# slothfulxtx/Texture-GS

Measured on AMD Instinct MI355X. Metric: fwd+bwd views/sec @800x800, 300k Gaussians + 1024^2 texture; HBM GB/s vs roofline, higher is better.
Workload: dtype f32; 1 GPU; c3: N=300000 Gaussians, cubemap 6x1024x1024x3 f32, 800x800, fwd+bwd, sh_degree 3; parallelism=views sharded dp1, view_pipeline=3 HIP streams, order=accumulate, forwards begun one view per stream ahead, grad_allreduce=none (1 GPU)

## Files before the change

### include/texgs_multiview.h

```cpp
#ifndef TEXGS_MULTIVIEW_H
#define TEXGS_MULTIVIEW_H

#include <stddef.h>
#include <stdint.h>

#include "texgs.h"

#ifdef __cplusplus
extern "C" {
#endif

#define TEXGS_SH_FLUSH_MAX_VIEWS 16

typedef struct TexGSShFlushView {
    const float* campos;
    const float* residue;
    int32_t sh_degree;
    int32_t sh_coeffs;
} TexGSShFlushView;

int texgs_sh_flush(int32_t N, int32_t K, const float* means3D, const float* shs, float* dL_dshs, float* dL_dmeans3D,
                   const TexGSShFlushView* views, int32_t count, void* stream);

#define TEXGS_BATCH_MAX_VIEWS 16

int texgs_preprocess_forward_views(const TexGSFrame* frames, const TexGSInputs* in, TexGSGeom* geoms, int32_t count, uint32_t* sums,
                                   void* stream);
int texgs_depth_sort_scan_views(const TexGSGeom* geoms, int32_t num_gaussians, int32_t count, void* stream);
int texgs_bin_sort_views(const TexGSFrame* frames, const TexGSGeom* geoms, TexGSBinning* bins, const TexGSImage* imgs, int32_t count,
                         void* stream);
int texgs_render_forward_binned(const TexGSFrame* frame, const TexGSInputs* in, const TexGSGeom* geom, const TexGSBinning* bin,
                                TexGSImage* img, void* stream);

#ifdef __cplusplus
}
#endif

#endif
```

### texture-gs_amd/csrc/abi.hip

```cpp
#include "common.h"
#include <stdio.h>
#include <stdlib.h>

#include <mutex>
#include <vector>

namespace {

thread_local char g_err[512] = "";

struct EvRec { int kid; hipEvent_t a, b; };
std::mutex g_prof_mu;
bool g_prof_on = false;
uint32_t g_prof_mask = 0xFFFFFFFFu;
std::vector<EvRec> g_prof_log;
std::vector<hipEvent_t> g_prof_free;

hipEvent_t prof_event() {
    if (!g_prof_free.empty()) { hipEvent_t e = g_prof_free.back(); g_prof_free.pop_back(); return e; }
    hipEvent_t e = nullptr;
    return hipEventCreate(&e) == hipSuccess ? e : nullptr;
}

struct ProfScope {
// ... 605 lines not shown
            if (!b.keys_unsorted || !b.keys_sorted || !b.point_list || !b.sort_temp) return fail_msg("NULL buffer in a view's TexGSBinning");
            if (b.sort_temp_bytes < sort_temp_bytes(b.num_rendered, T)) return fail_msg("sort_temp too small");
        }
        if ((imgs[v].tex_bin_count != nullptr) && frames[v].tex_res != frames[0].tex_res) return fail_msg("the views of a batch must have one tex_res");
    }
    hipStream_t s = (hipStream_t)stream;
    hipError_t st;
    const int nzw = 2 * (int)tex_bin_count(c.R);
    { ProfScope p(TEXGS_K_DUPLICATE, s); st = launch_bin_views(TEXGS_K_DUPLICATE, c, geoms, bins, imgs, count, nzw, s); }
    if (int r = launched("duplicate_with_keys (views)", st, s, frames[0].debug)) return r;
    { ProfScope p(TEXGS_K_SORT, s); st = launch_bin_views(TEXGS_K_SORT, c, geoms, bins, imgs, count, nzw, s); }
    if (int r = launched("tile sort (views)", st, s, frames[0].debug)) return r;
    { ProfScope p(TEXGS_K_RANGES, s); st = launch_bin_views(TEXGS_K_RANGES, c, geoms, bins, imgs, count, nzw, s); }
    return launched("tile_ranges (views)", st, s, frames[0].debug);
}

int texgs_render_forward_binned(const TexGSFrame* frame, const TexGSInputs* in, const TexGSGeom* geom, const TexGSBinning* bin,
                                TexGSImage* img, void* stream) {
    return render_forward_impl(frame, in, geom, bin, img, stream, true);
}

static int check_mlp(const TexGSMlp* m) {
    if (!m) return fail_msg("mlp is NULL");
    const char* what = nullptr;
    int v = 0;
    if (m->n_neurons != TEXGS_MLP_WIDTH) { what = "n_neurons must be 128"; v = m->n_neurons; }
    else if (m->n_hidden_layers < 1 || m->n_hidden_layers > TEXGS_MLP_MAX_HIDDEN_LAYERS) { what = "n_hidden_layers must be 1 or 2"; v = m->n_hidden_layers; }
    else if (m->n_in < 1 || m->n_in > TEXGS_MLP_WIDTH) { what = "n_in must be in [1,128]"; v = m->n_in; }
    else if (m->n_out < 1 || m->n_out > TEXGS_MLP_WIDTH) { what = "n_out must be in [1,128]"; v = m->n_out; }
    if (!what) return 0;
// ... 453 lines not shown
```

### texture-gs_amd/csrc/binning.hip

```cpp
#include "common.h"
#include <cstring>

namespace {

constexpr int RS_THREADS = 256;
constexpr int RS_MAX_BLOCKS = 1024;
constexpr int RS_GROUP = 32;
#ifndef RS_PER_MIN
#define RS_PER_MIN 512u
#endif

struct RadixTables {
    uint32_t* table;
    uint32_t* gtable;
};
constexpr size_t RS_ZERO_WORDS = (size_t)(RS_MAX_BLOCKS / RS_GROUP) * 256;

__device__ __forceinline__ uint32_t digit_of(uint64_t k, int shift, uint32_t mask) { return (uint32_t)(k >> shift) & mask; }

__device__ __forceinline__ void block_range(uint32_t n, uint32_t per, uint32_t& lo, uint32_t& hi) {
    lo = min(n, blockIdx.x * per);
    hi = min(n, lo + per);
}

// ... 17 lines not shown
    t.table[blockIdx.x * 256 + threadIdx.x] = c;
    if (c != 0u) atomicAdd(&t.gtable[(blockIdx.x / RS_GROUP) * 256 + threadIdx.x], c);
}

template <typename KEY>
__global__ void __launch_bounds__(RS_THREADS)
k_radix_count(const KEY* __restrict__ keys, const uint32_t* __restrict__ n_ptr, uint32_t n_max, uint32_t per, int shift,
              uint32_t mask, RadixTables t) {
    radix_count_body<KEY>(keys, n_ptr ? min(*n_ptr, n_max) : n_max, per, shift, mask, t);
}

template <typename KEY, int MODE>
__device__ __forceinline__ void radix_scatter_body(const KEY* __restrict__ keys_in, const uint32_t* __restrict__ vals_in, KEY* __restrict__ keys_out,
                uint32_t* __restrict__ vals_out, uint32_t n, uint32_t nblocks, uint32_t per, int shift,
                uint32_t mask, int bits, RadixTables t, const uint32_t* __restrict__ depth_rank,
                const uint32_t* __restrict__ id_rank) {
    __shared__ uint32_t s_wcnt[4][256];
    __shared__ uint32_t s_scan[256];
    uint32_t lo, hi;
    block_range(n, per, lo, hi);
    if (lo >= hi) return;
    const int tid = threadIdx.x, lane = tid & 63, wv = tid >> 6;
    constexpr int RB = 8;
    const uint32_t rows = (hi - lo + 63u) >> 6, rows_per_wave = (rows + 3u) >> 2;
    const uint32_t wlo = min(hi, lo + (uint32_t)wv * rows_per_wave * 64u), whi = min(hi, wlo + rows_per_wave * 64u);
    const bool single = (whi - wlo) <= 64u * RB;
    KEY kk[RB];
    uint32_t vv[RB];
    auto load_batch = [&](uint32_t b0) {
#pragma unroll
        for (int rr = 0; rr < RB; ++rr) {
// ... 36 lines not shown
#pragma unroll
        for (int rr = 0; rr < RB; ++rr)
            if (b0 + 64u * rr + lane < whi) atomicAdd(&s_wcnt[wv][digit_of(kk[rr], shift, mask)], 1u);
    }
    __syncthreads();
    {
        uint32_t run = before;
#pragma unroll
        for (int w = 0; w < 4; ++w) { const uint32_t c = s_wcnt[w][tid]; s_wcnt[w][tid] = run; run += c; }
    }
    __syncthreads();
    uint32_t* cur = s_wcnt[wv];
    for (uint32_t b0 = wlo; b0 < whi; b0 += 64u * RB) {
        if (!single) load_batch(b0);
        uint32_t dr[RB];
        if (MODE == 2) {
#pragma unroll
            for (int rr = 0; rr < RB; ++rr) {
                const bool have = b0 + 64u * rr + lane < whi;
                dr[rr] = have ? depth_rank[(uint32_t)kk[rr]] : 0u;
                vv[rr] = have ? id_rank[(uint32_t)kk[rr]] : 0u;
            }
        }
#pragma unroll
        for (int rr = 0; rr < RB; ++rr) {
            const uint32_t i = b0 + 64u * rr + lane;
            if (b0 + 64u * rr >= whi) break;
            const bool have = i < whi;
            const KEY k = kk[rr];
            const uint32_t d = have ? digit_of(k, shift, mask) : 0xFFFFFFFFu;
            unsigned long long peers = __ballot(have);
            for (int bt = 0; bt < bits; ++bt) {
                const unsigned long long m = __ballot((d >> bt) & 1u);
                peers &= ((d >> bt) & 1u) ? m : ~m;
            }
            uint32_t pos = 0u;
            if (have) {
                const uint32_t below = (uint32_t)__builtin_amdgcn_mbcnt_hi((uint32_t)(peers >> 32), __builtin_amdgcn_mbcnt_lo((uint32_t)peers, 0u));
                pos = cur[d] + below;
            }
            __builtin_amdgcn_wave_barrier();
            if (have && (peers >> lane) >> 1 == 0ull) cur[d] = pos + 1u;
            __builtin_amdgcn_wave_barrier();
            if (have) {
                if (MODE == 0) {
                    keys_out[pos] = k;
                    vals_out[pos] = vv[rr];
                } else if (MODE == 1) {
                    keys_out[pos] = k;
                } else {
                    keys_out[pos] = (KEY)(((uint64_t)k & 0xFFFFFFFF00000000ull) | (uint64_t)dr[rr]);
                    vals_out[pos] = vv[rr];
                }
            }
        }
    }
}

template <typename KEY, int MODE>
__global__ void __launch_bounds__(RS_THREADS)
k_radix_scatter(const KEY* __restrict__ keys_in, const uint32_t* __restrict__ vals_in, KEY* __restrict__ keys_out,
                uint32_t* __restrict__ vals_out, const uint32_t* __restrict__ n_ptr, uint32_t n_max, uint32_t per, int shift,
                uint32_t mask, int bits, RadixTables t, const uint32_t* __restrict__ depth_rank,
                const uint32_t* __restrict__ id_rank) {
    radix_scatter_body<KEY, MODE>(keys_in, vals_in, keys_out, vals_out, n_ptr ? min(*n_ptr, n_max) : n_max, gridDim.x, per, shift, mask,
                                  bits, t, depth_rank, id_rank);
// ... 413 lines not shown
    for (int k = 0; k < 9; ++k) { const int q = tid * per + k; v[k] = (k < per && q < nb1) ? bsum[q] : 0u; sum += v[k]; }
    uint32_t incl = sum;
#pragma unroll
    for (int d = 1; d < 64; d <<= 1) { const uint32_t o = (uint32_t)__shfl_up((int)incl, d, 64); if (lane >= d) incl += o; }
    if (lane == 63) s_w[wv] = incl;
    __syncthreads();
    uint32_t run = incl - sum;
    for (int w = 0; w < wv; ++w) run += s_w[w];
#pragma unroll
    for (int k = 0; k < 9; ++k) { const int q = tid * per + k; if (k < per && q < nb1) bsum[q] = run; run += v[k]; }
}

__global__ void __launch_bounds__(1024)
k_depth_prefix(const uint32_t* __restrict__ drange, uint32_t* __restrict__ bsum) { depth_prefix_body(drange, bsum); }

template <bool PRE>
__device__ __forceinline__ void duplicate_body(int N, int tiles_x, int T, const uint32_t* __restrict__ id_rank, const uint32_t* __restrict__ key_rank,
            const uint32_t* __restrict__ loc_rank, uint32_t* __restrict__ offs_rank, const uint32_t* __restrict__ drange, const uint32_t* __restrict__ gmap, const uint32_t* __restrict__ bsum,
            const uint32_t* __restrict__ tiles_touched, const uint2* __restrict__ rect, uint64_t* __restrict__ elems,
            uint2* __restrict__ ranges, uint32_t* __restrict__ zero_words, int num_zero_words) {
    __shared__ uint32_t s_pre[PRE ? 1 : DS_FUSED_GROUPS + 1];
    __shared__ uint32_t s_w[TG_BLOCK / 64];
    const int r = blockIdx.x * TG_BLOCK + threadIdx.x;
    for (int k = r; k < T; k += (int)gridDim.x * TG_BLOCK) ranges[k] = make_uint2(0u, 0u);
    for (int k = r; k < num_zero_words; k += (int)gridDim.x * TG_BLOCK) zero_words[k] = 0u;
    const uint32_t d_lo = drange[DR_LO], d_scale = drange[DR_SCALE], d_nb = drange[DR_NB];
    uint32_t my_group = 0u, my_off = 0u;
    if (r < N) { my_group = gmap[depth_bin(key_rank[r], d_lo, d_scale, d_nb)]; my_off = loc_rank[r]; }
    uint32_t my_pre = 0u;
    if constexpr (PRE) {
        if (r < N) my_pre = bsum[my_group];
    } else {
        const int tid = threadIdx.x, lane = tid & 63, wv = tid >> 6, nb1 = (int)drange[DR_GROUPS] + 1;
        for (int q = tid; q < nb1; q += TG_BLOCK) s_pre[q] = bsum[q];
        __syncthreads();
// ... 8 lines not shown
        uint32_t run = incl - sum;
        for (int w = 0; w < wv; ++w) run += s_w[w];
        for (int k = 0; k < per; ++k) { const int q = tid * per + k; if (q < nb1) { const uint32_t c = s_pre[q]; s_pre[q] = run; run += c; } }
        __syncthreads();
        my_pre = s_pre[my_group];
    }
    if (r >= N) return;
    uint32_t off = my_off + my_pre;
    offs_rank[r] = off;
    const uint32_t id = id_rank[r];
    if (tiles_touched[id] == 0u) return;
    const uint2 rc = rect[id];
    const uint32_t x0 = rc.x & 0xffffu, y0 = rc.x >> 16, x1 = rc.y & 0xffffu, y1 = rc.y >> 16;
    for (uint32_t y = y0; y < y1; ++y)
        for (uint32_t x = x0; x < x1; ++x)
            elems[off++] = ((uint64_t)(y * (uint32_t)tiles_x + x) << 32) | (uint64_t)(uint32_t)r;
}

template <bool PRE>
__global__ void __launch_bounds__(TG_BLOCK)
k_duplicate(int N, int tiles_x, int T, const uint32_t* __restrict__ id_rank, const uint32_t* __restrict__ key_rank,
            const uint32_t* __restrict__ loc_rank, uint32_t* __restrict__ offs_rank, const uint32_t* __restrict__ drange, const uint32_t* __restrict__ gmap, const uint32_t* __restrict__ bsum,
            const uint32_t* __restrict__ tiles_touched, const uint2* __restrict__ rect, uint64_t* __restrict__ elems,
            uint2* __restrict__ ranges, uint32_t* __restrict__ zero_words, int num_zero_words) {
    duplicate_body<PRE>(N, tiles_x, T, id_rank, key_rank, loc_rank, offs_rank, drange, gmap, bsum, tiles_touched, rect, elems, ranges,
                        zero_words, num_zero_words);
}

__device__ __forceinline__ void ranges_body(uint32_t D, const uint64_t* __restrict__ keys, uint2* __restrict__ ranges) {
    const uint32_t i = blockIdx.x * TG_BLOCK + threadIdx.x;
    if (i >= D) return;
    const uint32_t cur = (uint32_t)(keys[i] >> 32);
    if (i == 0) ranges[cur].x = 0;
    else {
        const uint32_t prev = (uint32_t)(keys[i - 1] >> 32);
        if (cur != prev) { ranges[prev].y = i; ranges[cur].x = i; }
    }
    if (i == D - 1) ranges[cur].y = D;
}

__global__ void __launch_bounds__(TG_BLOCK)
// ... 147 lines not shown
}

__global__ void __launch_bounds__(DS_THREADS)
k_depth_group_sort_views(BinViews a, int N, int gmax) {
    const BinView& w = a.v[blockIdx.y];
    const GaussScratch gs = gauss_scratch(w.scan_temp, N);
    depth_group_sort_body(N, gs.gpos, gs.drange, gs.pair_a, gs.key_b, gs.val_b, w.tiles_touched, gs.loc_b, gs.bsum, gmax);
}

__global__ void __launch_bounds__(1024)
k_depth_prefix_views(BinViews a, int N) {
    const GaussScratch gs = gauss_scratch(a.v[blockIdx.y].scan_temp, N);
    depth_prefix_body(gs.drange, gs.bsum);
}

template <bool PRE>
__global__ void __launch_bounds__(TG_BLOCK)
k_duplicate_views(BinViews a, int N, int tiles_x, int T, int num_zero_words) {
    const BinView& w = a.v[blockIdx.y];
    if (w.D == 0u) {
        for (int k = blockIdx.x * TG_BLOCK + threadIdx.x; k < T; k += (int)gridDim.x * TG_BLOCK) w.ranges[k] = make_uint2(0u, 0u);
        return;
    }
    const GaussScratch gs = gauss_scratch(w.scan_temp, N);
    duplicate_body<PRE>(N, tiles_x, T, gs.val_b, gs.key_b, gs.loc_b, w.offsets, gs.drange, gs.gmap, gs.bsum, w.tiles_touched, w.rect,
                        w.keys_unsorted, w.ranges, reinterpret_cast<uint32_t*>(w.sort_temp), num_zero_words);
}

__global__ void __launch_bounds__(RS_THREADS)
k_radix_count_views(BinViews a, int pass, int from_tmp, int shift, uint32_t mask) {
    const BinView& w = a.v[blockIdx.y];
    uint32_t blocks, per;
    pass_geometry(w.D, blocks, per);
    if (w.D == 0u || blockIdx.x >= blocks) return;
    radix_count_body<uint64_t>(from_tmp ? sort_tmp_of(w) : w.keys_unsorted, w.D, per, shift, mask,
                               tables_at(reinterpret_cast<uint32_t*>(w.sort_temp), pass, TILE_PASSES_MAX, 0));
}

template <int MODE>
__global__ void __launch_bounds__(RS_THREADS)
k_radix_scatter_views(BinViews a, int N, int pass, int from_tmp, int to_tmp, int shift, uint32_t mask, int bits) {
    const BinView& w = a.v[blockIdx.y];
    uint32_t blocks, per;
    pass_geometry(w.D, blocks, per);
    if (w.D == 0u || blockIdx.x >= blocks) return;
    const uint64_t* src = from_tmp ? sort_tmp_of(w) : w.keys_unsorted;
    const RadixTables t = tables_at(reinterpret_cast<uint32_t*>(w.sort_temp), pass, TILE_PASSES_MAX, 0);
    if (MODE == 2) {
        const GaussScratch gs = gauss_scratch(w.scan_temp, N);
        radix_scatter_body<uint64_t, 2>(src, nullptr, w.keys_sorted, w.point_list, w.D, blocks, per, shift, mask, bits, t, gs.key_b, gs.val_b);
    } else {
        radix_scatter_body<uint64_t, 1>(src, nullptr, to_tmp ? sort_tmp_of(w) : w.keys_unsorted, nullptr, w.D, blocks, per, shift, mask, bits, t,
                                        nullptr, nullptr);
    }
}

__global__ void __launch_bounds__(TG_BLOCK)
k_ranges_views(BinViews a) {
    const BinView& w = a.v[blockIdx.y];
    if (w.D != 0u) ranges_body(w.D, w.keys_sorted, w.ranges);
}

__global__ void __launch_bounds__(1024)
k_tile_order_views(BinViews a, uint32_t T, int num_zero_words) {
    const BinView& w = a.v[blockIdx.y];
    tile_order_body(T, w.ranges, w.tile_order, w.zero_words, w.zero_words ? num_zero_words : 0);
}

// ... 2 lines not shown
    memset(&a, 0, sizeof(a));
    for (int v = 0; v < count; ++v) {
        BinView& w = a.v[v];
        w.depth = reinterpret_cast<const uint32_t*>(g[v].depth); w.tiles_touched = g[v].tiles_touched;
        w.rect = reinterpret_cast<const uint2*>(g[v].rect); w.offsets = g[v].offsets; w.scan_temp = g[v].scan_temp;
        if (b) {
            w.keys_unsorted = b[v].keys_unsorted; w.keys_sorted = b[v].keys_sorted; w.point_list = b[v].point_list;
            w.ranges = reinterpret_cast<uint2*>(b[v].ranges); w.tile_order = b[v].tile_order; w.sort_temp = b[v].sort_temp;
            w.D = b[v].num_rendered;
        }
        if (img) w.zero_words = img[v].tex_bin_count;
    }
    return a;
}

}

hipError_t launch_depth_sort_scan_views(const TexGSGeom* g, int N, int count, hipStream_t s) {
    if (N <= 0 || count <= 0) return hipSuccess;
    const BinViews a = bin_views(g, nullptr, nullptr, count);
    const int nblk = (N + TG_BLOCK - 1) / TG_BLOCK;
    const int blocks = (N + DS_PER - 1) / DS_PER;
    const int lb = depth_log2_bins(N);
    const int gmax = depth_max_groups(N, 1 << lb);
    hipLaunchKernelGGL(k_depth_count_views, dim3(blocks, count), dim3(DS_THREADS), 0, s, a, N, nblk, lb);
    hipLaunchKernelGGL(k_depth_scatter_views, dim3(blocks, count), dim3(DS_THREADS), 0, s, a, N, nblk, lb);
    hipLaunchKernelGGL(k_depth_group_sort_views, dim3(gmax + (N + (int)DS_COPY - 1) / (int)DS_COPY, count), dim3(DS_THREADS), 0, s, a, N, gmax);
    if (gmax > DS_FUSED_GROUPS) hipLaunchKernelGGL(k_depth_prefix_views, dim3(1, count), dim3(1024), 0, s, a, N);
    return hipGetLastError();
}

hipError_t launch_bin_views(int stage, const CamConst& c, const TexGSGeom* g, const TexGSBinning* b, const TexGSImage* img, int count,
                            int num_zero_words, hipStream_t s) {
    if (c.N <= 0 || count <= 0) return hipSuccess;
    const BinViews a = bin_views(g, b, img, count);
    const uint32_t T = (uint32_t)(c.tiles_x * c.tiles_y);
    uint32_t dmax = 0u;
    for (int v = 0; v < count; ++v) dmax = b[v].num_rendered > dmax ? b[v].num_rendered : dmax;
    const int nblocks = (c.N + TG_BLOCK - 1) / TG_BLOCK;
    const bool pre = depth_max_groups(c.N, 1 << depth_log2_bins(c.N)) > DS_FUSED_GROUPS;
    const int hdr = (int)(zero_header_bytes(TILE_PASSES_MAX, 0) / 4);
    if (stage == TEXGS_K_DUPLICATE) {
        if (pre) hipLaunchKernelGGL(k_duplicate_views<true>, dim3(nblocks, count), dim3(TG_BLOCK), 0, s, a, c.N, c.tiles_x, (int)T, hdr);
        else hipLaunchKernelGGL(k_duplicate_views<false>, dim3(nblocks, count), dim3(TG_BLOCK), 0, s, a, c.N, c.tiles_x, (int)T, hdr);
    }
    if (stage == TEXGS_K_SORT && dmax > 0u) {
        const int tb = tile_bits(T);
        const int npass = (tb + 7) / 8;
        if (npass > TILE_PASSES_MAX) return hipErrorInvalidValue;
        uint32_t blocks = 1u;
        for (int v = 0; v < count; ++v) {
            uint32_t bv, per;
            pass_geometry(b[v].num_rendered, bv, per);
            blocks = bv > blocks ? bv : blocks;
        }
        int from_tmp = 0, shift = 32, left = tb;
        for (int pass = 0; pass < npass; ++pass) {
            const int bits = (left + (npass - pass) - 1) / (npass - pass);
            const uint32_t mask = (1u << bits) - 1u;
            hipLaunchKernelGGL(k_radix_count_views, dim3(blocks, count), dim3(RS_THREADS), 0, s, a, pass, from_tmp, shift, mask);
            if (pass == npass - 1) {
                hipLaunchKernelGGL(k_radix_scatter_views<2>, dim3(blocks, count), dim3(RS_THREADS), 0, s, a, c.N, pass, from_tmp, 0, shift, mask, bits);
            } else {
                const int to_tmp = from_tmp ? 0 : 1;
                hipLaunchKernelGGL(k_radix_scatter_views<1>, dim3(blocks, count), dim3(RS_THREADS), 0, s, a, c.N, pass, from_tmp, to_tmp, shift, mask, bits);
                from_tmp = to_tmp;
            }
            shift += bits; left -= bits;
        }
    }
    if (stage == TEXGS_K_RANGES) {
        if (dmax > 0u) hipLaunchKernelGGL(k_ranges_views, dim3((dmax + TG_BLOCK - 1) / TG_BLOCK, count), dim3(TG_BLOCK), 0, s, a);
        hipLaunchKernelGGL(k_tile_order_views, dim3(1, count), dim3(1024), 0, s, a, T, num_zero_words);
    }
    return hipGetLastError();
}

hipError_t launch_depth_sort_scan(const TexGSGeom* g, int N, hipStream_t s) {
    if (N <= 0) return hipSuccess;
    const GaussScratch gs = gauss_scratch(g->scan_temp, N);
    const int nblk = (N + TG_BLOCK - 1) / TG_BLOCK;
    const int blocks = (N + DS_PER - 1) / DS_PER;
// ... 111 lines not shown
```

### texture-gs_amd/csrc/common.h

```cpp
#pragma once
#include <hip/hip_runtime.h>
#include <stdint.h>
#include "texgs.h"
#include "texgs_optim.h"
#include "texgs_multiview.h"
#include "texgs_mlp.h"
#include "texgs_present.h"
#include "texgs_ingest.h"
#include "texgs_surface.h"
#include "texgs_lpips.h"
#include "texgs_lpips_grad.h"
#include "texgs_params.h"
#include "texgs_retexture.h"

#define TG_NEAR_Z        0.2f
#define TG_LOWPASS       0.3f
#define TG_FRUSTUM_CLAMP 1.3f
#define TG_ALPHA_MAX     0.99f
#define TG_ALPHA_MIN     (1.0f / 255.0f)
#define TG_T_EPS         1e-4f
#define TG_PLANE_EPS     5e-2f
#define TG_DEN_MIN       0.2f
#define TG_MA_MIN        1e-20f
#define TG_SH_C0         0.28209479177387814f
// ... 39 lines not shown
hipError_t launch_sh_flush(int N, int K, const float* means3D, const float* shs, float* dL_dshs, float* dL_dmeans3D,
                           const TexGSShFlushView* views, int count, hipStream_t s);
hipError_t launch_mark_visible(const TexGSFrame* f, const float* means3D, uint8_t* visible, hipStream_t s);
hipError_t launch_depth_sort_scan(const TexGSGeom* g, int N, hipStream_t s);
uint32_t* bin_block_sums_ptr(const TexGSGeom* g, int N);
uint32_t* bin_header_ptr(const TexGSGeom* g, int N, int* words);
size_t scan_temp_bytes(int N);
size_t sort_temp_bytes(uint32_t D, uint32_t T);
hipError_t launch_duplicate(const CamConst& c, const TexGSGeom* g, TexGSBinning* b, hipStream_t s);
hipError_t launch_sort(const CamConst& c, const TexGSGeom* g, TexGSBinning* b, hipStream_t s);
hipError_t launch_ranges(const CamConst& c, TexGSBinning* b, uint32_t* zero_words, int num_zero_words, hipStream_t s);
hipError_t launch_preprocess_fwd_views(const TexGSFrame* f, const TexGSInputs* in, TexGSGeom* g, int count, uint32_t* sums, hipStream_t s);
hipError_t launch_depth_sort_scan_views(const TexGSGeom* g, int N, int count, hipStream_t s);
hipError_t launch_bin_views(int stage, const CamConst& c, const TexGSGeom* g, const TexGSBinning* b, const TexGSImage* img, int count,
                            int num_zero_words, hipStream_t s);
hipError_t launch_render_fwd(const CamConst& c, const TexGSFrame* f, const TexGSInputs* in, const TexGSGeom* g,
                       const TexGSBinning* b, TexGSImage* img, hipStream_t s);
size_t tex_bin_count(int R);
bool tex_bins_enabled(const CamConst& c, const TexGSInputs* in, const TexGSImage* img, const TexGSGrads* gr);
hipError_t launch_texgrad_reduce(const CamConst& c, const TexGSImage* img, TexGSGrads* gr, hipStream_t s);
hipError_t launch_render_bwd(const CamConst& c, const TexGSFrame* f, const TexGSInputs* in, const TexGSGeom* g,
                       const TexGSBinning* b, const TexGSImage* img, TexGSGrads* gr, hipStream_t s);
hipError_t launch_rgb_alpha_loss(const float* image, const float* gt_image, const float* alpha, const float* gt_alpha, int H,
                          int W, float lambda_dssim, float lambda_alpha, float* scratch, float* sums, float* d_image,
                          float* d_alpha, hipStream_t s);
hipError_t launch_selftest_waveops(const float* seed128, float* out576, hipStream_t s);
hipError_t launch_geom_losses(const float* norm, const float* gt_norm, const float* gt_image, const float* mask, const float* depth,
                       const float* gt_depth, int H, int W, float lambda_norm, float lambda_smooth, float gamma,
                       float lambda_depth, float* sums, float* d_norm, float* d_depth, hipStream_t s);
hipError_t launch_norm_from_depth(const float* depth, const float* viewmatrix, float tanfovx, float tanfovy, int H, int W, float threshold,
// ... 67 lines not shown
```

### texture-gs_amd/csrc/preprocess.hip

```cpp
#include "common.h"
#include <cstring>

namespace {

struct Frame {
    float V[16];
    float P[16];
    float cam[3];
};

__device__ __forceinline__ Frame load_frame(const float* vm, const float* pm, const float* cp) {
    Frame f;
#pragma unroll
    for (int i = 0; i < 16; ++i) { f.V[i] = vm[i]; f.P[i] = pm[i]; }
    f.cam[0] = cp[0]; f.cam[1] = cp[1]; f.cam[2] = cp[2];
    return f;
}

struct Geo {
    bool  valid;
    float m[3], t[3];
    float hx, hy, hw, pw, xy[2];
    float q[4], s[3], R[9], M[9], S[6];
    float txc, tyc; bool clx, cly;
// ... 670 lines not shown
    OUT(TEXGS_ACC_ROTATIONS, d_rots[4 * i + 2], 2.0f * (-2.0f * y * dR[0] + x * dR[1] + r * dR[2] + x * dR[3] + z * dR[5] - r * dR[6] + z * dR[7] - 2.0f * y * dR[8]));
    OUT(TEXGS_ACC_ROTATIONS, d_rots[4 * i + 3], 2.0f * (-2.0f * z * dR[0] - r * dR[1] + x * dR[2] + r * dR[3] - 2.0f * z * dR[4] + y * dR[5] + x * dR[6] + y * dR[7]));
    }
#undef OUT
    }
    if constexpr (!DEFER) if (d_shs) {
        if (na == 0 || (live && !visible)) {
            if (live) for (int k = 0; k < row; ++k) s_sh[threadIdx.x * row + k] = 0.f;
        }
        __syncthreads();
        if (accumulate & TEXGS_ACC_SHS) sh_rows_out<BLOCK, true>(d_shs + first, s_sh, count, vec);
        else sh_rows_out<BLOCK, false>(d_shs + first, s_sh, count, vec);
    }
}

constexpr int FL_BLOCK = 256;
constexpr int FL_MAX = TEXGS_SH_FLUSH_MAX_VIEWS;

struct ShFlushArgs {
    TexGSShFlushView v[FL_MAX];
    int32_t count;
};

__global__ void __launch_bounds__(FL_BLOCK)
k_sh_flush(ShFlushArgs a, int N, int K, const float* __restrict__ means, const float* __restrict__ shs,
           float* __restrict__ d_shs, float* __restrict__ d_means) {
    extern __shared__ __attribute__((aligned(16))) float s_row[];
    const int i = blockIdx.x * FL_BLOCK + threadIdx.x;
    const bool live = i < N;
    const int row = 3 * K;
    const size_t first = (size_t)blockIdx.x * FL_BLOCK * row;
    const int count = (int)min((size_t)FL_BLOCK * row, (size_t)N * row - first);
    const bool vec = (((size_t)d_shs) & 15) == 0;
    for (int k = threadIdx.x; k < count; k += FL_BLOCK) s_row[k] = shs[first + k];
    __syncthreads();
    float sp[45];
#pragma unroll
    for (int k = 0; k < 45; ++k) sp[k] = (live && k < row) ? s_row[threadIdx.x * row + k] : 0.f;
    __syncthreads();
    for (int k = threadIdx.x; k < count; k += FL_BLOCK) s_row[k] = d_shs[first + k];
    __syncthreads();
    if (live) {
        const float m[3] = {means[3 * i + 0], means[3 * i + 1], means[3 * i + 2]};
        float* gp = s_row + threadIdx.x * row;
        float dm[3] = {d_means[3 * i + 0], d_means[3 * i + 1], d_means[3 * i + 2]};
        bool any = false;
        for (int v = 0; v < a.count; ++v) {
            const float* __restrict__ res = a.v[v].residue;
            const float v0 = res[3 * i + 0], v1 = res[3 * i + 1], v2 = res[3 * i + 2];
            const int deg = a.v[v].sh_degree;
            const int na = deg > 0 ? sh_active(deg, K) : 0;
            if ((v0 == 0.f && v1 == 0.f && v2 == 0.f) || na == 0) continue;
            const float* __restrict__ cp = a.v[v].campos;
            const float cam[3] = {cp[0], cp[1], cp[2]};
            float raw[3], dir[3];
            const float dlen = view_direction(m, cam, raw, dir);
            float b[15], bx[15], by[15], bz[15];
#pragma unroll
            for (int k = 0; k < 15; ++k) { b[k] = 0.f; bx[k] = 0.f; by[k] = 0.f; bz[k] = 0.f; }
            sh_basis(deg, dir[0], dir[1], dir[2], b);
            sh_basis_grad(deg, dir[0], dir[1], dir[2], bx, by, bz);
            float ddx = 0.f, ddy = 0.f, ddz = 0.f;
#pragma unroll
            for (int k = 0; k < 15; ++k) {
                if (k < na) {
                    const float w = sp[3 * k + 0] * v0 + sp[3 * k + 1] * v1 + sp[3 * k + 2] * v2;
                    ddx += bx[k] * w; ddy += by[k] * w; ddz += bz[k] * w;
                    gp[3 * k + 0] = gp[3 * k + 0] + b[k] * v0; gp[3 * k + 1] = gp[3 * k + 1] + b[k] * v1;
                    gp[3 * k + 2] = gp[3 * k + 2] + b[k] * v2;
                }
            }
            const float dd = dir[0] * ddx + dir[1] * ddy + dir[2] * ddz;
            dm[0] += (ddx - dir[0] * dd) / dlen;
            dm[1] += (ddy - dir[1] * dd) / dlen;
            dm[2] += (ddz - dir[2] * dd) / dlen;
            any = true;
        }
        if (any) { d_means[3 * i + 0] = dm[0]; d_means[3 * i + 1] = dm[1]; d_means[3 * i + 2] = dm[2]; }
    }
    __syncthreads();
    sh_rows_out<FL_BLOCK, false>(d_shs + first, s_row, count, vec);
}

__global__ void __launch_bounds__(TG_BLOCK)
k_mark_visible(int N, const float* __restrict__ vm, const float* __restrict__ means, uint8_t* __restrict__ visible) {
    const int i = blockIdx.x * TG_BLOCK + threadIdx.x;
    if (i >= N) return;
    const float tz = vm[2] * means[3 * i] + vm[6] * means[3 * i + 1] + vm[10] * means[3 * i + 2] + vm[14];
    visible[i] = tz > TG_NEAR_Z ? 1 : 0;
}

}

hipError_t launch_preprocess_fwd(const CamConst& c, const TexGSFrame* f, const TexGSInputs* in, TexGSGeom* g, hipStream_t s) {
    if (c.N <= 0) return hipSuccess;
    const int blocks = (c.N + TG_BLOCK - 1) / TG_BLOCK;
// ... 48 lines not shown
        const size_t lds = gr->dL_dshs ? (size_t)K8_BLOCK * 3 * c.sh_coeffs * sizeof(float) : 0;
        if (in->cov3D_precomp) K8_LAUNCH(true, false, K8_BLOCK, lds); else K8_LAUNCH(false, false, K8_BLOCK, lds);
    }
#undef K8_LAUNCH
    return hipGetLastError();
}

hipError_t launch_sh_flush(int N, int K, const float* means3D, const float* shs, float* dL_dshs, float* dL_dmeans3D,
                           const TexGSShFlushView* views, int count, hipStream_t s) {
    if (count < 0 || count > FL_MAX) return hipErrorInvalidValue;
    if (N <= 0 || count == 0) return hipSuccess;
    ShFlushArgs a;
    for (int k = 0; k < FL_MAX; ++k) a.v[k] = k < count ? views[k] : TexGSShFlushView{nullptr, nullptr, 0, 0};
    a.count = count;
    const size_t lds = (size_t)FL_BLOCK * 3 * K * sizeof(float);
    hipLaunchKernelGGL(k_sh_flush, dim3((N + FL_BLOCK - 1) / FL_BLOCK), dim3(FL_BLOCK), lds, s, a, N, K, means3D, shs, dL_dshs, dL_dmeans3D);
    return hipGetLastError();
}

hipError_t launch_mark_visible(const TexGSFrame* f, const float* means3D, uint8_t* visible, hipStream_t s) {
    if (f->num_gaussians <= 0) return hipSuccess;
    const int blocks = (f->num_gaussians + TG_BLOCK - 1) / TG_BLOCK;
    hipLaunchKernelGGL(k_mark_visible, dim3(blocks), dim3(TG_BLOCK), 0, s, f->num_gaussians, f->viewmatrix, means3D, visible);
    return hipGetLastError();
}
```

### texture-gs_amd/texgs/multiview.py

```python
import contextlib
import ctypes as C
from typing import List, Sequence

import torch

SH_FLUSH_MAX_VIEWS = 16


class ShFlushView(C.Structure):
    _fields_ = [("campos", C.c_void_p), ("residue", C.c_void_p), ("sh_degree", C.c_int32), ("sh_coeffs", C.c_int32)]


SH_FLUSH_SIGNATURE = (C.c_int, [C.c_int32, C.c_int32, C.c_void_p, C.c_void_p, C.c_void_p, C.c_void_p, C.POINTER(ShFlushView), C.c_int32,
                                C.c_void_p])
_sh_flush_fn = None


def sh_flush_entry():
    global _sh_flush_fn
    if _sh_flush_fn is None:
        from . import _lib
        lib = _lib.load()
        if not hasattr(lib, "texgs_sh_flush"):
            raise RuntimeError(f"libtexgs.so at {_lib.LIB_PATH} does not export texgs_sh_flush; rebuild it with "
# ... 2 lines not shown
        fn.restype, fn.argtypes = SH_FLUSH_SIGNATURE
        _sh_flush_fn = fn
    return _sh_flush_fn


BATCH_MAX_VIEWS = 16


def views_signatures():
    from . import _lib
    P, vp, i32 = C.POINTER, C.c_void_p, C.c_int32
    return {
        "texgs_preprocess_forward_views": (C.c_int, [P(_lib.Frame), P(_lib.Inputs), P(_lib.Geom), i32, vp, vp]),
        "texgs_depth_sort_scan_views": (C.c_int, [P(_lib.Geom), i32, i32, vp]),
        "texgs_bin_sort_views": (C.c_int, [P(_lib.Frame), P(_lib.Geom), P(_lib.Binning), P(_lib.Image), i32, vp]),
        "texgs_render_forward_binned": (C.c_int, [P(_lib.Frame), P(_lib.Inputs), P(_lib.Geom), P(_lib.Binning), P(_lib.Image), vp]),
    }


_views_fns = None


def views_entries():
    global _views_fns
    if _views_fns is None:
        from types import SimpleNamespace
        from . import _lib
        lib = _lib.load()
        fns = {}
        for name, (restype, argtypes) in views_signatures().items():
# ... 384 lines not shown
```

Measured before the change: 1065 views/s.

## Pack batched tile-sort keys into 32 bits and register-stage SH flush inputs

When the tile bits plus rank bits fit in 32 bits, the batched binning path now writes 32-bit tile|rank elements. It radix-sorts those instead of 64-bit keys and widens them to 64-bit keys only in the final scatter, which halves sort traffic. The SH flush kernel is templated on the view count and vector alignment. It prefetches SH rows, gradients, residues and camera positions into registers with float4 loads before staging through LDS. The costs are more register pressure and extra kernel variants, and the packed path depends on N and the tile count fitting in 32 bits.

```diff
diff --git a/include/texgs_multiview.h b/include/texgs_multiview.h
--- a/include/texgs_multiview.h
+++ b/include/texgs_multiview.h
@@ -29,6 +29,7 @@
 int texgs_depth_sort_scan_views(const TexGSGeom* geoms, int32_t num_gaussians, int32_t count, void* stream);
 int texgs_bin_sort_views(const TexGSFrame* frames, const TexGSGeom* geoms, TexGSBinning* bins, const TexGSImage* imgs, int32_t count,
                          void* stream);
+int texgs_batch_packed_elems(int32_t on);
 int texgs_render_forward_binned(const TexGSFrame* frame, const TexGSInputs* in, const TexGSGeom* geom, const TexGSBinning* bin,
                                 TexGSImage* img, void* stream);
 
diff --git a/texture-gs_amd/csrc/abi.hip b/texture-gs_amd/csrc/abi.hip
--- a/texture-gs_amd/csrc/abi.hip
+++ b/texture-gs_amd/csrc/abi.hip
@@ -643,6 +643,8 @@
     { ProfScope p(TEXGS_K_RANGES, s); st = launch_bin_views(TEXGS_K_RANGES, c, geoms, bins, imgs, count, nzw, s); }
     return launched("tile_ranges (views)", st, s, frames[0].debug);
 }
+
+int texgs_batch_packed_elems(int32_t on) { return set_batch_packed_elems(on); }
 
 int texgs_render_forward_binned(const TexGSFrame* frame, const TexGSInputs* in, const TexGSGeom* geom, const TexGSBinning* bin,
                                 TexGSImage* img, void* stream) {
diff --git a/texture-gs_amd/csrc/binning.hip b/texture-gs_amd/csrc/binning.hip
--- a/texture-gs_amd/csrc/binning.hip
+++ b/texture-gs_amd/csrc/binning.hip
@@ -55,7 +55,8 @@
 __device__ __forceinline__ void radix_scatter_body(const KEY* __restrict__ keys_in, const uint32_t* __restrict__ vals_in, KEY* __restrict__ keys_out,
                 uint32_t* __restrict__ vals_out, uint32_t n, uint32_t nblocks, uint32_t per, int shift,
                 uint32_t mask, int bits, RadixTables t, const uint32_t* __restrict__ depth_rank,
-                const uint32_t* __restrict__ id_rank) {
+                const uint32_t* __restrict__ id_rank, int rank_bits = 0) {
+    static_assert(MODE != 3 || sizeof(KEY) == 4, "MODE 3 splits 32-bit elements");
     __shared__ uint32_t s_wcnt[4][256];
     __shared__ uint32_t s_scan[256];
     uint32_t lo, hi;
@@ -122,12 +123,14 @@
     for (uint32_t b0 = wlo; b0 < whi; b0 += 64u * RB) {
         if (!single) load_batch(b0);
         uint32_t dr[RB];
-        if (MODE == 2) {
+        if (MODE == 2 || MODE == 3) {
+            const uint32_t rank_mask = MODE == 3 ? (1u << rank_bits) - 1u : 0xFFFFFFFFu;
 #pragma unroll
             for (int rr = 0; rr < RB; ++rr) {
                 const bool have = b0 + 64u * rr + lane < whi;
-                dr[rr] = have ? depth_rank[(uint32_t)kk[rr]] : 0u;
-                vv[rr] = have ? id_rank[(uint32_t)kk[rr]] : 0u;
+                const uint32_t rank = (uint32_t)kk[rr] & rank_mask;
+                dr[rr] = have ? depth_rank[rank] : 0u;
+                vv[rr] = have ? id_rank[rank] : 0u;
             }
         }
 #pragma unroll
@@ -156,8 +159,11 @@
                     vals_out[pos] = vv[rr];
                 } else if (MODE == 1) {
                     keys_out[pos] = k;
+                } else if (MODE == 2) {
+                    keys_out[pos] = (KEY)(((uint64_t)k & 0xFFFFFFFF00000000ull) | (uint64_t)dr[rr]);
+                    vals_out[pos] = vv[rr];
                 } else {
-                    keys_out[pos] = (KEY)(((uint64_t)k & 0xFFFFFFFF00000000ull) | (uint64_t)dr[rr]);
+                    reinterpret_cast<uint64_t*>(keys_out)[pos] = ((uint64_t)((uint32_t)k >> rank_bits) << 32) | (uint64_t)dr[rr];
                     vals_out[pos] = vv[rr];
                 }
             }
@@ -601,11 +607,11 @@
 __global__ void __launch_bounds__(1024)
 k_depth_prefix(const uint32_t* __restrict__ drange, uint32_t* __restrict__ bsum) { depth_prefix_body(drange, bsum); }
 
-template <bool PRE>
+template <bool PRE, typename ELEM>
 __device__ __forceinline__ void duplicate_body(int N, int tiles_x, int T, const uint32_t* __restrict__ id_rank, const uint32_t* __restrict__ key_rank,
             const uint32_t* __restrict__ loc_rank, uint32_t* __restrict__ offs_rank, const uint32_t* __restrict__ drange, const uint32_t* __restrict__ gmap, const uint32_t* __restrict__ bsum,
-            const uint32_t* __restrict__ tiles_touched, const uint2* __restrict__ rect, uint64_t* __restrict__ elems,
-            uint2* __restrict__ ranges, uint32_t* __restrict__ zero_words, int num_zero_words) {
+            const uint32_t* __restrict__ tiles_touched, const uint2* __restrict__ rect, ELEM* __restrict__ elems,
+            uint2* __restrict__ ranges, uint32_t* __restrict__ zero_words, int num_zero_words, int eshift) {
     __shared__ uint32_t s_pre[PRE ? 1 : DS_FUSED_GROUPS + 1];
     __shared__ uint32_t s_w[TG_BLOCK / 64];
     const int r = blockIdx.x * TG_BLOCK + threadIdx.x;
@@ -644,7 +650,7 @@
     const uint32_t x0 = rc.x & 0xffffu, y0 = rc.x >> 16, x1 = rc.y & 0xffffu, y1 = rc.y >> 16;
     for (uint32_t y = y0; y < y1; ++y)
         for (uint32_t x = x0; x < x1; ++x)
-            elems[off++] = ((uint64_t)(y * (uint32_t)tiles_x + x) << 32) | (uint64_t)(uint32_t)r;
+            elems[off++] = ((ELEM)(y * (uint32_t)tiles_x + x) << eshift) | (ELEM)(uint32_t)r;
 }
 
 template <bool PRE>
@@ -653,8 +659,8 @@
             const uint32_t* __restrict__ loc_rank, uint32_t* __restrict__ offs_rank, const uint32_t* __restrict__ drange, const uint32_t* __restrict__ gmap, const uint32_t* __restrict__ bsum,
             const uint32_t* __restrict__ tiles_touched, const uint2* __restrict__ rect, uint64_t* __restrict__ elems,
             uint2* __restrict__ ranges, uint32_t* __restrict__ zero_words, int num_zero_words) {
-    duplicate_body<PRE>(N, tiles_x, T, id_rank, key_rank, loc_rank, offs_rank, drange, gmap, bsum, tiles_touched, rect, elems, ranges,
-                        zero_words, num_zero_words);
+    duplicate_body<PRE, uint64_t>(N, tiles_x, T, id_rank, key_rank, loc_rank, offs_rank, drange, gmap, bsum, tiles_touched, rect, elems, ranges,
+                                  zero_words, num_zero_words, 32);
 }
 
 __device__ __forceinline__ void ranges_body(uint32_t D, const uint64_t* __restrict__ keys, uint2* __restrict__ ranges) {
@@ -832,44 +838,51 @@
     depth_prefix_body(gs.drange, gs.bsum);
 }
 
-template <bool PRE>
+template <bool PRE, bool PACKED>
 __global__ void __launch_bounds__(TG_BLOCK)
-k_duplicate_views(BinViews a, int N, int tiles_x, int T, int num_zero_words) {
+k_duplicate_views(BinViews a, int N, int tiles_x, int T, int num_zero_words, int rank_bits) {
     const BinView& w = a.v[blockIdx.y];
     if (w.D == 0u) {
         for (int k = blockIdx.x * TG_BLOCK + threadIdx.x; k < T; k += (int)gridDim.x * TG_BLOCK) w.ranges[k] = make_uint2(0u, 0u);
         return;
     }
     const GaussScratch gs = gauss_scratch(w.scan_temp, N);
-    duplicate_body<PRE>(N, tiles_x, T, gs.val_b, gs.key_b, gs.loc_b, w.offsets, gs.drange, gs.gmap, gs.bsum, w.tiles_touched, w.rect,
-                        w.keys_unsorted, w.ranges, reinterpret_cast<uint32_t*>(w.sort_temp), num_zero_words);
-}
-
+    if constexpr (PACKED)
+        duplicate_body<PRE, uint32_t>(N, tiles_x, T, gs.val_b, gs.key_b, gs.loc_b, w.offsets, gs.drange, gs.gmap, gs.bsum, w.tiles_touched, w.rect,
+                                      reinterpret_cast<uint32_t*>(w.keys_unsorted), w.ranges, reinterpret_cast<uint32_t*>(w.sort_temp),
+                                      num_zero_words, rank_bits);
+    else
+        duplicate_body<PRE, uint64_t>(N, tiles_x, T, gs.val_b, gs.key_b, gs.loc_b, w.offsets, gs.drange, gs.gmap, gs.bsum, w.tiles_touched, w.rect,
+                                      w.keys_unsorted, w.ranges, reinterpret_cast<uint32_t*>(w.sort_temp), num_zero_words, 32);
+}
+
+template <typename KEY>
 __global__ void __launch_bounds__(RS_THREADS)
 k_radix_count_views(BinViews a, int pass, int from_tmp, int shift, uint32_t mask) {
     const BinView& w = a.v[blockIdx.y];
     uint32_t blocks, per;
     pass_geometry(w.D, blocks, per);
     if (w.D == 0u || blockIdx.x >= blocks) return;
-    radix_count_body<uint64_t>(from_tmp ? sort_tmp_of(w) : w.keys_unsorted, w.D, per, shift, mask,
-                               tables_at(reinterpret_cast<uint32_t*>(w.sort_temp), pass, TILE_PASSES_MAX, 0));
-}
-
-template <int MODE>
+    radix_count_body<KEY>(reinterpret_cast<const KEY*>(from_tmp ? sort_tmp_of(w) : w.keys_unsorted), w.D, per, shift, mask,
+                          tables_at(reinterpret_cast<uint32_t*>(w.sort_temp), pass, TILE_PASSES_MAX, 0));
+}
+
+template <typename KEY, int MODE>
 __global__ void __launch_bounds__(RS_THREADS)
-k_radix_scatter_views(BinViews a, int N, int pass, int from_tmp, int to_tmp, int shift, uint32_t mask, int bits) {
+k_radix_scatter_views(BinViews a, int N, int pass, int from_tmp, int to_tmp, int shift, uint32_t mask, int bits, int rank_bits) {
     const BinView& w = a.v[blockIdx.y];
     uint32_t blocks, per;
     pass_geometry(w.D, blocks, per);
     if (w.D == 0u || blockIdx.x >= blocks) return;
-    const uint64_t* src = from_tmp ? sort_tmp_of(w) : w.keys_unsorted;
+    const KEY* src = reinterpret_cast<const KEY*>(from_tmp ? sort_tmp_of(w) : w.keys_unsorted);
     const RadixTables t = tables_at(reinterpret_cast<uint32_t*>(w.sort_temp), pass, TILE_PASSES_MAX, 0);
-    if (MODE == 2) {
+    if (MODE == 2 || MODE == 3) {
         const GaussScratch gs = gauss_scratch(w.scan_temp, N);
-        radix_scatter_body<uint64_t, 2>(src, nullptr, w.keys_sorted, w.point_list, w.D, blocks, per, shift, mask, bits, t, gs.key_b, gs.val_b);
+        radix_scatter_body<KEY, MODE>(src, nullptr, reinterpret_cast<KEY*>(w.keys_sorted), w.point_list, w.D, blocks, per, shift, mask, bits, t,
+                                      gs.key_b, gs.val_b, rank_bits);
     } else {
-        radix_scatter_body<uint64_t, 1>(src, nullptr, to_tmp ? sort_tmp_of(w) : w.keys_unsorted, nullptr, w.D, blocks, per, shift, mask, bits, t,
-                                        nullptr, nullptr);
+        radix_scatter_body<KEY, 1>(src, nullptr, reinterpret_cast<KEY*>(to_tmp ? sort_tmp_of(w) : w.keys_unsorted), nullptr, w.D, blocks, per,
+                                   shift, mask, bits, t, nullptr, nullptr);
     }
 }
 
@@ -902,7 +915,17 @@
     return a;
 }
 
-}
+int g_batch_packed = 1;
+
+inline int rank_bits_of(int N) {
+    int bits = 1;
+    while (bits < 31 && (1u << bits) < (uint32_t)N) ++bits;
+    return bits;
+}
+
+}
+
+int set_batch_packed_elems(int on) { const int was = g_batch_packed; g_batch_packed = on ? 1 : 0; return was; }
 
 hipError_t launch_depth_sort_scan_views(const TexGSGeom* g, int N, int count, hipStream_t s) {
     if (N <= 0 || count <= 0) return hipSuccess;
@@ -928,12 +951,16 @@
     const int nblocks = (c.N + TG_BLOCK - 1) / TG_BLOCK;
     const bool pre = depth_max_groups(c.N, 1 << depth_log2_bins(c.N)) > DS_FUSED_GROUPS;
     const int hdr = (int)(zero_header_bytes(TILE_PASSES_MAX, 0) / 4);
+    const int tb = tile_bits(T);
+    const int rb = rank_bits_of(c.N);
+    const bool packed = g_batch_packed && tb + rb <= 32;
     if (stage == TEXGS_K_DUPLICATE) {
-        if (pre) hipLaunchKernelGGL(k_duplicate_views<true>, dim3(nblocks, count), dim3(TG_BLOCK), 0, s, a, c.N, c.tiles_x, (int)T, hdr);
-        else hipLaunchKernelGGL(k_duplicate_views<false>, dim3(nblocks, count), dim3(TG_BLOCK), 0, s, a, c.N, c.tiles_x, (int)T, hdr);
+#define K3V_LAUNCH(PRE, PACKED) hipLaunchKernelGGL((k_duplicate_views<PRE, PACKED>), dim3(nblocks, count), dim3(TG_BLOCK), 0, s, a, c.N, c.tiles_x, (int)T, hdr, rb)
+        if (packed) { if (pre) K3V_LAUNCH(true, true); else K3V_LAUNCH(false, true); }
+        else { if (pre) K3V_LAUNCH(true, false); else K3V_LAUNCH(false, false); }
+#undef K3V_LAUNCH
     }
     if (stage == TEXGS_K_SORT && dmax > 0u) {
-        const int tb = tile_bits(T);
         const int npass = (tb + 7) / 8;
         if (npass > TILE_PASSES_MAX) return hipErrorInvalidValue;
         uint32_t blocks = 1u;
@@ -942,18 +969,22 @@
             pass_geometry(b[v].num_rendered, bv, per);
             blocks = bv > blocks ? bv : blocks;
         }
-        int from_tmp = 0, shift = 32, left = tb;
+        int from_tmp = 0, shift = packed ? rb : 32, left = tb;
         for (int pass = 0; pass < npass; ++pass) {
             const int bits = (left + (npass - pass) - 1) / (npass - pass);
             const uint32_t mask = (1u << bits) - 1u;
-            hipLaunchKernelGGL(k_radix_count_views, dim3(blocks, count), dim3(RS_THREADS), 0, s, a, pass, from_tmp, shift, mask);
+            if (packed) hipLaunchKernelGGL(k_radix_count_views<uint32_t>, dim3(blocks, count), dim3(RS_THREADS), 0, s, a, pass, from_tmp, shift, mask);
+            else hipLaunchKernelGGL(k_radix_count_views<uint64_t>, dim3(blocks, count), dim3(RS_THREADS), 0, s, a, pass, from_tmp, shift, mask);
+#define K4V_LAUNCH(KEY, MODE, TO) hipLaunchKernelGGL((k_radix_scatter_views<KEY, MODE>), dim3(blocks, count), dim3(RS_THREADS), 0, s, a, c.N, pass, from_tmp, TO, \
+                                                     shift, mask, bits, rb)
             if (pass == npass - 1) {
-                hipLaunchKernelGGL(k_radix_scatter_views<2>, dim3(blocks, count), dim3(RS_THREADS), 0, s, a, c.N, pass, from_tmp, 0, shift, mask, bits);
+                if (packed) K4V_LAUNCH(uint32_t, 3, 0); else K4V_LAUNCH(uint64_t, 2, 0);
             } else {
                 const int to_tmp = from_tmp ? 0 : 1;
-                hipLaunchKernelGGL(k_radix_scatter_views<1>, dim3(blocks, count), dim3(RS_THREADS), 0, s, a, c.N, pass, from_tmp, to_tmp, shift, mask, bits);
+                if (packed) K4V_LAUNCH(uint32_t, 1, to_tmp); else K4V_LAUNCH(uint64_t, 1, to_tmp);
                 from_tmp = to_tmp;
             }
+#undef K4V_LAUNCH
             shift += bits; left -= bits;
         }
     }
diff --git a/texture-gs_amd/csrc/common.h b/texture-gs_amd/csrc/common.h
--- a/texture-gs_amd/csrc/common.h
+++ b/texture-gs_amd/csrc/common.h
@@ -77,6 +77,7 @@
 hipError_t launch_depth_sort_scan_views(const TexGSGeom* g, int N, int count, hipStream_t s);
 hipError_t launch_bin_views(int stage, const CamConst& c, const TexGSGeom* g, const TexGSBinning* b, const TexGSImage* img, int count,
                             int num_zero_words, hipStream_t s);
+int set_batch_packed_elems(int on);
 hipError_t launch_render_fwd(const CamConst& c, const TexGSFrame* f, const TexGSInputs* in, const TexGSGeom* g,
                        const TexGSBinning* b, TexGSImage* img, hipStream_t s);
 size_t tex_bin_count(int R);
diff --git a/texture-gs_amd/csrc/preprocess.hip b/texture-gs_amd/csrc/preprocess.hip
--- a/texture-gs_amd/csrc/preprocess.hip
+++ b/texture-gs_amd/csrc/preprocess.hip
@@ -708,14 +708,62 @@
     }
 }
 
-constexpr int FL_BLOCK = 256;
+#ifndef FL_BLOCK_THREADS
+#define FL_BLOCK_THREADS 256
+#endif
+constexpr int FL_BLOCK = FL_BLOCK_THREADS;
 constexpr int FL_MAX = TEXGS_SH_FLUSH_MAX_VIEWS;
+constexpr int FL_ROW_MAX = 48;
 
 struct ShFlushArgs {
     TexGSShFlushView v[FL_MAX];
     int32_t count;
 };
 
+struct FlRows {
+    float w[FL_ROW_MAX];
+    float tail;
+};
+
+template <bool VEC>
+__device__ __forceinline__ void fl_rows_load(const float* __restrict__ g, int count, FlRows& q) {
+    const int tid = (int)threadIdx.x;
+    q.tail = 0.f;
+    if constexpr (VEC) {
+        const int n4 = count >> 2;
+        const float4* __restrict__ g4 = reinterpret_cast<const float4*>(g);
+#pragma unroll
+        for (int u = 0; u < FL_ROW_MAX / 4; ++u) {
+            const int k = tid + u * FL_BLOCK;
+            const float4 x = (k < n4) ? g4[k] : make_float4(0.f, 0.f, 0.f, 0.f);
+            q.w[4 * u + 0] = x.x; q.w[4 * u + 1] = x.y; q.w[4 * u + 2] = x.z; q.w[4 * u + 3] = x.w;
+        }
+        if (tid < (count & 3)) q.tail = g[4 * n4 + tid];
+    } else {
+#pragma unroll
+        for (int j = 0; j < FL_ROW_MAX; ++j) { const int k = tid + j * FL_BLOCK; q.w[j] = (k < count) ? g[k] : 0.f; }
+    }
+}
+
+template <bool VEC>
+__device__ __forceinline__ void fl_rows_to_lds(const FlRows& q, float* s, int count) {
+    const int tid = (int)threadIdx.x;
+    if constexpr (VEC) {
+        const int n4 = count >> 2;
+        float4* s4 = reinterpret_cast<float4*>(s);
+#pragma unroll
+        for (int u = 0; u < FL_ROW_MAX / 4; ++u) {
+            const int k = tid + u * FL_BLOCK;
+            if (k < n4) s4[k] = make_float4(q.w[4 * u + 0], q.w[4 * u + 1], q.w[4 * u + 2], q.w[4 * u + 3]);
+        }
+        if (tid < (count & 3)) s[4 * n4 + tid] = q.tail;
+    } else {
+#pragma unroll
+        for (int j = 0; j < FL_ROW_MAX; ++j) { const int k = tid + j * FL_BLOCK; if (k < count) s[k] = q.w[j]; }
+    }
+}
+
+template <int NV, bool VEC>
 __global__ void __launch_bounds__(FL_BLOCK)
 k_sh_flush(ShFlushArgs a, int N, int K, const float* __restrict__ means, const float* __restrict__ shs,
            float* __restrict__ d_shs, float* __restrict__ d_means) {
@@ -725,28 +773,49 @@
     const int row = 3 * K;
     const size_t first = (size_t)blockIdx.x * FL_BLOCK * row;
     const int count = (int)min((size_t)FL_BLOCK * row, (size_t)N * row - first);
-    const bool vec = (((size_t)d_shs) & 15) == 0;
-    for (int k = threadIdx.x; k < count; k += FL_BLOCK) s_row[k] = shs[first + k];
+    FlRows q_sh, q_g;
+    fl_rows_load<VEC>(shs + first, count, q_sh);
+    fl_rows_load<VEC>(d_shs + first, count, q_g);
+    float res[NV][3], cams[NV][3];
+#pragma unroll
+    for (int v = 0; v < NV; ++v) {
+        const bool have = v < a.count;
+        const float* __restrict__ rp = a.v[v].residue;
+        const float* __restrict__ cp = a.v[v].campos;
+#pragma unroll
+        for (int c = 0; c < 3; ++c) {
+            res[v][c] = (have && live) ? rp[3 * (size_t)i + c] : 0.f;
+            cams[v][c] = have ? cp[c] : 0.f;
+        }
+    }
+    float m[3] = {0.f, 0.f, 0.f}, dm[3] = {0.f, 0.f, 0.f};
+    if (live) {
+#pragma unroll
+        for (int c = 0; c < 3; ++c) { m[c] = means[3 * (size_t)i + c]; dm[c] = d_means[3 * (size_t)i + c]; }
+    }
+    fl_rows_to_lds<VEC>(q_sh, s_row, count);
     __syncthreads();
     float sp[45];
 #pragma unroll
     for (int k = 0; k < 45; ++k) sp[k] = (live && k < row) ? s_row[threadIdx.x * row + k] : 0.f;
     __syncthreads();
-    for (int k = threadIdx.x; k < count; k += FL_BLOCK) s_row[k] = d_shs[first + k];
+    fl_rows_to_lds<VEC>(q_g, s_row, count);
     __syncthreads();
     if (live) {
-        const float m[3] = {means[3 * i + 0], means[3 * i + 1], means[3 * i + 2]};
         float* gp = s_row + threadIdx.x * row;
-        float dm[3] = {d_means[3 * i + 0], d_means[3 * i + 1], d_means[3 * i + 2]};
         bool any = false;
+#pragma unroll 1
         for (int v = 0; v < a.count; ++v) {
-            const float* __restrict__ res = a.v[v].residue;
-            const float v0 = res[3 * i + 0], v1 = res[3 * i + 1], v2 = res[3 * i + 2];
+            const float v0 = res[0][0], v1 = res[0][1], v2 = res[0][2];
+            const float cam[3] = {cams[0][0], cams[0][1], cams[0][2]};
+#pragma unroll
+            for (int k = 0; k + 1 < NV; ++k) {
+#pragma unroll
+                for (int c = 0; c < 3; ++c) { res[k][c] = res[k + 1][c]; cams[k][c] = cams[k + 1][c]; }
+            }
             const int deg = a.v[v].sh_degree;
             const int na = deg > 0 ? sh_active(deg, K) : 0;
             if ((v0 == 0.f && v1 == 0.f && v2 == 0.f) || na == 0) continue;
-            const float* __restrict__ cp = a.v[v].campos;
-            const float cam[3] = {cp[0], cp[1], cp[2]};
             float raw[3], dir[3];
             const float dlen = view_direction(m, cam, raw, dir);
             float b[15], bx[15], by[15], bz[15];
@@ -773,7 +842,7 @@
         if (any) { d_means[3 * i + 0] = dm[0]; d_means[3 * i + 1] = dm[1]; d_means[3 * i + 2] = dm[2]; }
     }
     __syncthreads();
-    sh_rows_out<FL_BLOCK, false>(d_shs + first, s_row, count, vec);
+    sh_rows_out<FL_BLOCK, false>(d_shs + first, s_row, count, VEC);
 }
 
 __global__ void __launch_bounds__(TG_BLOCK)
@@ -852,7 +921,13 @@
     for (int k = 0; k < FL_MAX; ++k) a.v[k] = k < count ? views[k] : TexGSShFlushView{nullptr, nullptr, 0, 0};
     a.count = count;
     const size_t lds = (size_t)FL_BLOCK * 3 * K * sizeof(float);
-    hipLaunchKernelGGL(k_sh_flush, dim3((N + FL_BLOCK - 1) / FL_BLOCK), dim3(FL_BLOCK), lds, s, a, N, K, means3D, shs, dL_dshs, dL_dmeans3D);
+    static_assert(FL_MAX == 16, "two flavours: up to 8 and up to 16 views' residues in registers");
+    const dim3 grid((N + FL_BLOCK - 1) / FL_BLOCK);
+    const bool vec = ((((size_t)shs) | ((size_t)dL_dshs)) & 15) == 0;
+#define FL_LAUNCH(NV, VEC) hipLaunchKernelGGL((k_sh_flush<NV, VEC>), grid, dim3(FL_BLOCK), lds, s, a, N, K, means3D, shs, dL_dshs, dL_dmeans3D)
+    if (count <= 8) { if (vec) FL_LAUNCH(8, true); else FL_LAUNCH(8, false); }
+    else { if (vec) FL_LAUNCH(16, true); else FL_LAUNCH(16, false); }
+#undef FL_LAUNCH
     return hipGetLastError();
 }
 
diff --git a/texture-gs_amd/texgs/multiview.py b/texture-gs_amd/texgs/multiview.py
--- a/texture-gs_amd/texgs/multiview.py
+++ b/texture-gs_amd/texgs/multiview.py
@@ -40,6 +40,7 @@
         "texgs_preprocess_forward_views": (C.c_int, [P(_lib.Frame), P(_lib.Inputs), P(_lib.Geom), i32, vp, vp]),
         "texgs_depth_sort_scan_views": (C.c_int, [P(_lib.Geom), i32, i32, vp]),
         "texgs_bin_sort_views": (C.c_int, [P(_lib.Frame), P(_lib.Geom), P(_lib.Binning), P(_lib.Image), i32, vp]),
+        "texgs_batch_packed_elems": (C.c_int, [i32]),
         "texgs_render_forward_binned": (C.c_int, [P(_lib.Frame), P(_lib.Inputs), P(_lib.Geom), P(_lib.Binning), P(_lib.Image), vp]),
     }
 
```

New measurement: 1046 views/s, median of 2. About the same (-1.8%).
